# zailaiyiwan123/NOVA_pointcloud

Measured on AMD Instinct MI355X. Metric: generated points/sec/node, NOVA-d48w1024 @2048 pts, 64-step sample, higher is better.
Workload: dtype bf16; 1 GPU; d48w1024_2048pts_b32; ar_steps=64, diffusion_steps=25, batch_per_gpu=32, global_batch=32, guidance=cfg 2-pass, process_group=none

## Files before the change

include/nova_hip.h:

```cpp
#ifndef NOVA_HIP_H_
#define NOVA_HIP_H_

#ifdef __cplusplus
extern "C" {
#endif

#define NOVA_HIP_VERSION 405

typedef enum { NOVA_F32 = 0, NOVA_BF16 = 1, NOVA_F16 = 2 } nova_dtype;
typedef enum { NOVA_ACT_NONE = 0, NOVA_ACT_GELU_ERF = 1, NOVA_ACT_SILU = 2 } nova_act;
typedef enum {
  NOVA_OK = 0,
  NOVA_ERR_ARG = -1,
  NOVA_ERR_SHAPE = -2,
  NOVA_ERR_LAUNCH = -3,
  NOVA_ERR_DEVICE = -4
} nova_status;

int nova_version(void);
const char* nova_last_error(void);
int nova_check_device(void);

#define NOVA_PROF_SLOTS 10
int nova_prof_enable(int on);
int nova_prof_collect(double* ms, double* work, long long* launches, int slots);

int nova_debug_force_gemm_tile(int tile);

int nova_debug_set_attn_variant(int variant);

int nova_debug_set_graphs(int on);
int nova_debug_graph_stats(long* captures, long* replays);
int nova_debug_drop_graphs(void);

int nova_gemm_bias_act(const void* A, const void* W, const float* bias, void* out, int M, int N, int K, int act,
                       int dtype, void* stream);

int nova_quantize_rows_fp8(const void* x_bf16, void* out_fp8, float* scale, long long rows, int D, void* stream);
int nova_gemm_fp8_bias_act(const void* A8, const float* a_scale, const void* W8, const float* w_scale, const float* bias,
                           void* out_bf16, int M, int N, int K, int act, void* stream);

int nova_qkv_rope(const void* x, const void* Wqkv, const float* bias, const float* rope, void* qkv, int S, int L, int D,
                  int heads, int rope_batch, int dtype, void* stream);

int nova_qkv_rope_cols(const void* x, const void* W, const float* bias, const float* rope, void* out, int M, int N, int K,
                       int L, int rope_batch, int head_dim, int rope_cols, int dtype, void* stream);

int nova_rope_table(const float* pos, const long long* ids, float* rope, int nb, int pad, int n_tok, int n_pos, int hd,
                    const float* inv_freq, void* stream);

int nova_attn_fwd(const void* q, const void* k, const void* v, void* o, int S, int heads, int Lq, int Lk, int head_dim,
                  long q_row_stride, long kv_row_stride, long o_row_stride, float scale, int dtype, void* stream);

int nova_attn_fwd_lse(const void* q_scaled, const void* k, const void* v, void* o, float* lse, int S, int heads, int L,
                      int head_dim, long qkv_row_stride, long o_row_stride, const int* key_limit, void* stream);
int nova_attn_bwd(const void* q_scaled, const void* k, const void* v, const void* o, const void* d_o, const float* lse,
                  float* delta_scratch, void* dq, void* dk, void* dv, int S, int heads, int L, int head_dim,
                  long qkv_row_stride, long o_row_stride, long do_row_stride, long dqkv_row_stride, float scale,
                  const int* key_limit, void* stream);

int nova_attn_cross_fwd_lse(const void* q_scaled, const void* k, const void* v, void* o, float* lse, int S, int heads, int Lq, int Lk,
                            int head_dim, long q_row_stride, long kv_row_stride, long o_row_stride, const int* key_limit,
                            void* stream);
int nova_attn_cross_bwd(const void* q_scaled, const void* k, const void* v, const void* o, const void* d_o, const float* lse,
                        float* delta_scratch, void* dq, void* dk, void* dv, int S, int heads, int Lq, int Lk, int head_dim,
                        long q_row_stride, long kv_row_stride, long o_row_stride, long do_row_stride, long dq_row_stride,
                        long dkv_row_stride, float scale, const int* key_limit, void* stream);

int nova_act_fwd(const void* x, void* y, long long n, int kind, int dtype, void* stream);
int nova_act_bwd(const void* x, const void* dy, void* dx, long long n, int kind, int dtype, void* stream);

int nova_row_norm_bwd(const void* x, const void* dy, const float* gamma, const float* beta, const void* mod, long mod_ld,
                      int scale_off, int shift_off, int gate_off, void* dx, void* dmod, float* dgamma_part, float* dbeta_part,
                      int parts, long rows, int D, float eps, int dtype, void* stream);

int nova_row_norm(const void* in, void* out, const float* gamma, const float* beta, const void* mod, long mod_ld,
                  int scale_off, int shift_off, int gate_off, const void* res, const int* gather, long rows, int D,
                  float eps, int dtype, void* stream);

int nova_row_norm_chain(const void* g, const void* x, const float* gamma, const float* beta, const void* mod, long mod_ld,
// ... 227 lines not shown
```

nova_pointcloud_amd/csrc/capi.hip:

```cpp
#include <cstdarg>
#include <cstdio>
#include <cstring>
#include <atomic>
#include <cmath>
#include <mutex>
#include <utility>
#include <vector>
#include "common.h"
#include "nova_internal.h"

namespace nova {

static thread_local char g_err[512] = "";

int set_error(int code, const char* fmt, ...) {
  va_list ap;
  va_start(ap, fmt);
  vsnprintf(g_err, sizeof(g_err), fmt, ap);
  va_end(ap);
  return code;
}

int check_launch(const char* what) {
  const hipError_t e = hipGetLastError();
  if (e == hipSuccess) return 0;
  return set_error(NOVA_ERR_LAUNCH, "%s: %s", what, hipGetErrorString(e));
}

struct ProfRec { hipEvent_t a, b; int slot; double work; };
static std::atomic<bool> g_prof_on{false};
static std::mutex g_prof_mu;
static std::vector<ProfRec> g_prof;
static std::vector<std::pair<hipEvent_t, hipEvent_t>> g_prof_pool;

bool prof_enabled() { return g_prof_on.load(std::memory_order_relaxed); }

ProfScope::ProfScope(int slot, double work, hipStream_t s) : idx(-1), st(s) {
  if (!prof_enabled()) return;
  std::lock_guard<std::mutex> lk(g_prof_mu);
  ProfRec r;
  if (!g_prof_pool.empty()) {
    r.a = g_prof_pool.back().first;
    r.b = g_prof_pool.back().second;
    g_prof_pool.pop_back();
  } else if (hipEventCreate(&r.a) != hipSuccess || hipEventCreate(&r.b) != hipSuccess) {
    return;
  }
  r.slot = slot;
  r.work = work;
  (void)hipEventRecord(r.a, st);
  g_prof.push_back(r);
  idx = (int)g_prof.size() - 1;
}
ProfScope::~ProfScope() {
  if (idx < 0) return;
  std::lock_guard<std::mutex> lk(g_prof_mu);
  if (idx < (int)g_prof.size()) (void)hipEventRecord(g_prof[idx].b, st);
}

static thread_local bool g_walk_rev = false;
void walk_reverse(bool on) { g_walk_rev = on; }
bool walk_is_reverse() { return g_walk_rev; }
#ifdef NOVA_EXPERIMENTS
static int g_walk_alternate = 1;
void walk_set_alternate(int on) { g_walk_alternate = on; }
#else
constexpr int g_walk_alternate = 1;
#endif
struct Walk {
  int k = 0;
  void next() { walk_reverse(g_walk_alternate && (k++ & 1)); }
  ~Walk() { walk_reverse(false); }
};
}

using namespace nova;

extern "C" {

int nova_version(void) { return NOVA_HIP_VERSION; }
const char* nova_last_error(void) { return g_err; }

int nova_check_device(void) {
  int dev = -1;
  if (hipGetDevice(&dev) != hipSuccess) return set_error(NOVA_ERR_DEVICE, "no HIP device");
  hipDeviceProp_t prop;
  if (hipGetDeviceProperties(&prop, dev) != hipSuccess) return set_error(NOVA_ERR_DEVICE, "hipGetDeviceProperties failed");
  if (strncmp(prop.gcnArchName, "gfx950", 6) != 0)
    return set_error(NOVA_ERR_DEVICE, "device %d is %s; libnova_hip is built for gfx950 only", dev, prop.gcnArchName);
  return 0;
}

int nova_debug_force_gemm_tile(int tile) {
  NOVA_REQUIRE(gemm_force_tile(tile) == 0, NOVA_ERR_ARG,
               "force_gemm_tile: this build knows 0 (auto), 16 (small-M kernel; 161 / 162 / 164 with 16 / 32 / 64 rows per workgroup), 64 / 128 (the small-M tile kernels), 256 (persistent), 257 (one tile per workgroup) and 258 (persistent, prologue form); experiment codes need the NOVA_EXPERIMENTS build");
  return 0;
}

int nova_prof_enable(int on) {
  g_prof_on.store(on != 0);
  return 0;
}

int nova_prof_collect(double* ms, double* work, long long* launches, int slots) {
  NOVA_REQUIRE(ms && work && launches && slots >= PROF_SLOTS, NOVA_ERR_ARG, "prof_collect: need %d slots", PROF_SLOTS);
  for (int i = 0; i < slots; ++i) { ms[i] = 0; work[i] = 0; launches[i] = 0; }
  std::lock_guard<std::mutex> lk(g_prof_mu);
  for (auto& r : g_prof) {
    float t = 0.f;
    if (hipEventSynchronize(r.b) == hipSuccess && hipEventElapsedTime(&t, r.a, r.b) == hipSuccess) {
      ms[r.slot] += t;
      work[r.slot] += r.work;
      launches[r.slot] += 1;
    }
    g_prof_pool.emplace_back(r.a, r.b);
  }
  g_prof.clear();
  return 0;
}

int nova_gemm_bias_act(const void* A, const void* W, const float* bias, void* out, int M, int N, int K, int act,
                       int dtype, void* stream) {
  NOVA_REQUIRE(!bad_dtype(dtype), NOVA_ERR_ARG, "gemm: bad dtype %d", dtype);
  NOVA_REQUIRE(M == 0 || (A && W && out), NOVA_ERR_ARG, "gemm: null pointer");
  return gemm_bias_act(A, W, bias, out, M, N, K, act, dtype, (hipStream_t)stream);
}

int nova_quantize_rows_fp8(const void* x, void* out, float* scale, long long rows, int D, void* stream) {
  NOVA_REQUIRE(rows <= 0 || (x && out && scale), NOVA_ERR_ARG, "quantize_rows_fp8: null pointer");
  return quantize_rows_fp8(x, out, scale, (long)rows, D, (hipStream_t)stream);
}

int nova_gemm_fp8_bias_act(const void* A8, const float* a_scale, const void* W8, const float* w_scale, const float* bias,
                           void* out, int M, int N, int K, int act, void* stream) {
  NOVA_REQUIRE(M <= 0 || (A8 && a_scale && W8 && w_scale && out), NOVA_ERR_ARG, "gemm_fp8: null pointer");
  NOVA_REQUIRE(act >= NOVA_ACT_NONE && act <= NOVA_ACT_SILU, NOVA_ERR_ARG, "gemm_fp8: bad activation %d", act);
  return gemm256_fp8_launch({.A8 = A8, .sa = a_scale, .W8 = W8, .sw = w_scale, .C = out, .M = M, .N = N, .K = K, .epi = act, .e = epi_bias(bias)},
                            (hipStream_t)stream);
}

int nova_qkv_rope(const void* x, const void* Wqkv, const float* bias, const float* rope, void* qkv, int S, int L, int D,
                  int heads, int rope_batch, int dtype, void* stream) {
  NOVA_REQUIRE(!bad_dtype(dtype), NOVA_ERR_ARG, "qkv_rope: bad dtype %d", dtype);
  NOVA_REQUIRE(S * L == 0 || (x && Wqkv && qkv), NOVA_ERR_ARG, "qkv_rope: null pointer");
  return gemm_qkv_rope(x, Wqkv, bias, rope, qkv, S, L, D, heads, rope_batch, dtype, (hipStream_t)stream);
}

int nova_qkv_rope_cols(const void* x, const void* W, const float* bias, const float* rope, void* out, int M, int N, int K,
// ... 295 lines not shown
```

nova_pointcloud_amd/csrc/denoise.hip:

```cpp
#include <atomic>
#include <cstdlib>
#include <string>
#include <unordered_map>
#include <utility>
#include "nova_internal.h"

namespace nova {

enum class Echo { none, energy, rows };

struct DenoiseCall {
  const nova_decoder* dec;
  const void *zc, *temb;
  float* x;
  const nova_sampler_step* sched;
  const float *noise, *echo_noise;
  float renorm;
  Echo echo;
  float *echo_energy, *echo_rows;
  int Ne, steps, S, B, n, P, D;
  void *ws_a, *ws_u, *ws_h, *ws_f, *ws_g, *ws_mod;
  float* ws_v;
  int mod_steps, dtype;
  hipStream_t st;
// ... 103 lines not shown
      epoch = now;
    }
    auto it = execs.find(key);
    if (it == execs.end()) {
      if (execs.size() >= 2048) clear();
      hipGraphExec_t exec = nullptr;
      hipError_t e = hipStreamBeginCapture(st, hipStreamCaptureModeThreadLocal);
      if (e == hipSuccess) {
        const int rc = launches();
        hipGraph_t graph = nullptr;
        e = hipStreamEndCapture(st, &graph);
        if (e == hipSuccess && graph && rc == 0) e = hipGraphInstantiate(&exec, graph, nullptr, nullptr, 0);
        if (graph) (void)hipGraphDestroy(graph);
        if (rc != 0) return rc;
      }
      if (e != hipSuccess || !exec) {
        (void)hipGetLastError();
        return launches();
      }
      it = execs.emplace(std::move(key), exec).first;
      ++captures;
    } else {
      ++replays;
    }
    const hipError_t el = hipGraphLaunch(it->second, st);
    NOVA_REQUIRE(el == hipSuccess, NOVA_ERR_LAUNCH, "decoder_denoise: hipGraphLaunch failed: %s", hipGetErrorString(el));
    return 0;
  }
};
static thread_local DecoderGraphs g_dec_graphs;
static std::atomic<int> g_graphs_on{-1};

static bool graphs_enabled() {
  int v = g_graphs_on.load(std::memory_order_relaxed);
  if (v < 0) {
    const char* e = getenv("NOVA_GRAPHS");
    g_graphs_on.store(v = (e && e[0] == '0') ? 0 : 1);
  }
  return v != 0;
}

template <typename T> static void key_put(std::string& k, const T& v) { k.append(reinterpret_cast<const char*>(&v), sizeof(T)); }

static std::string graph_key(const DenoiseCall& c) {
  std::string key;
  key.reserve(512 + sizeof(nova_sampler_step) * c.steps + sizeof(nova_mlp_block) * c.dec->depth);
  key_put(key, c.dec->depth);
  const void* dec_ptrs[] = {c.dec->adaln_w, c.dec->adaln_b, c.dec->patch_w, c.dec->patch_b, c.dec->head_w, c.dec->head_b};
  key_put(key, dec_ptrs);
  for (int b = 0; b < c.dec->depth; ++b) key_put(key, c.dec->blocks[b]);
  for (int i = 0; i < c.steps; ++i) key_put(key, c.sched[i]);
  const void* ptrs[] = {c.zc, c.temb, c.x, c.ws_a, c.ws_u, c.ws_h, c.ws_f, c.ws_g, c.ws_mod, (const void*)c.st};
  key_put(key, ptrs);
  const int ints[] = {c.steps, c.S, c.B, c.n, c.P, c.D, c.mod_steps, c.dtype, walk_is_reverse() ? 1 : 0, gemm_forced_tile(), skinny_forced_row_blocks()};
  key_put(key, ints);
  return key;
}

static int denoise(const DenoiseCall& c) {
  if (c.n == 0 || c.B == 0) return 0;
  if (c.echo != Echo::none || !graphs_enabled() || prof_enabled() || c.noise != nullptr || c.steps < 2) return denoise_launches(c);
  return g_dec_graphs.run(graph_key(c), c.st, [&c] { return denoise_launches(c); });
}

}

using namespace nova;

extern "C" {

int nova_debug_set_graphs(int on) {
  g_graphs_on.store(on ? 1 : 0);
  if (!on) {
    g_graph_epoch.fetch_add(1);
    g_dec_graphs.clear();
  }
  return 0;
}

int nova_debug_drop_graphs(void) {
  g_dec_graphs.clear();
  return 0;
}

int nova_debug_graph_stats(long* captures, long* replays) {
  if (captures) *captures = g_dec_graphs.captures;
  if (replays) *replays = g_dec_graphs.replays;
  return 0;
}

int nova_decoder_denoise(const nova_decoder* dec, const void* zc, const void* temb, float* x, const nova_sampler_step* sched,
                         const float* noise, float renorm, float* echo_energy, int steps, int S, int B, int n, int P, int D,
                         void* ws_a, void* ws_u, void* ws_h, void* ws_f, void* ws_g, void* ws_mod, float* ws_v, int mod_steps,
                         int dtype, void* stream) {
  const DenoiseCall c{dec, zc, temb, x, sched, noise, nullptr, renorm, renorm < 1.0f ? Echo::energy : Echo::none, echo_energy, nullptr, 0,
                      steps, S, B, n, P, D, ws_a, ws_u, ws_h, ws_f, ws_g, ws_mod, ws_v, mod_steps, dtype, (hipStream_t)stream};
  NOVA_TRY(check_call("decoder_denoise", c));
  NOVA_REQUIRE(c.echo == Echo::none || (echo_energy && ws_v), NOVA_ERR_ARG, "decoder_denoise: renorm needs echo_energy and ws_v");
  return denoise(c);
}

int nova_decoder_denoise_echo(const nova_decoder* dec, const void* zc, const void* temb, float* x, const nova_sampler_step* sched,
                              const float* noise, float renorm, float* echo_rows, const float* echo_noise, int Ne, int steps, int S, int B,
                              int n, int P, int D, void* ws_a, void* ws_u, void* ws_h, void* ws_f, void* ws_g, void* ws_mod, float* ws_v,
                              int mod_steps, int dtype, void* stream) {
  const DenoiseCall c{dec, zc, temb, x, sched, noise, echo_noise, renorm, Echo::rows, nullptr, echo_rows, Ne,
                      steps, S, B, n, P, D, ws_a, ws_u, ws_h, ws_f, ws_g, ws_mod, ws_v, mod_steps, dtype, (hipStream_t)stream};
// ... 8 lines not shown
```

nova_pointcloud_amd/csrc/gemm.hip:

```cpp
#include <cstdlib>
#include "common.h"
#include "nova_internal.h"

namespace nova {

constexpr int ROWB = 128;

template <typename T> struct Frag;
template <> struct Frag<bf16_t> { u4v v; };
template <> struct Frag<f16_t> { u4v v; };
template <> struct Frag<float> { f4v v; };

__device__ __forceinline__ f4v mma(const Frag<bf16_t>& w, const Frag<bf16_t>& a, f4v c) { return Half16<bf16_t>::mfma16(w.v, a.v, c); }
__device__ __forceinline__ f4v mma(const Frag<f16_t>& w, const Frag<f16_t>& a, f4v c) { return Half16<f16_t>::mfma16(w.v, a.v, c); }
__device__ __forceinline__ f4v mma(const Frag<float>& w, const Frag<float>& a, f4v c) {
#pragma unroll
  for (int j = 0; j < 4; ++j) c = __builtin_amdgcn_mfma_f32_16x16x4f32(w.v[j], a.v[j], c, 0, 0, 0);
  return c;
}

template <typename T>
__device__ __forceinline__ Frag<T> lds_frag(const char* tile, int row, int chunk) {
  const int phys = chunk ^ ((row >> 1) & 7);
  Frag<T> f;
  f.v = *reinterpret_cast<const decltype(f.v)*>(tile + row * ROWB + phys * 16);
  return f;
}

#ifndef NOVA_GEMM64_STAGES
#define NOVA_GEMM64_STAGES 2
#endif
template <typename T, int EPI, int F = 4>
__global__ __launch_bounds__(256, 2) void gemm_kernel(const T* __restrict__ A, const T* __restrict__ W,
                                                       T* __restrict__ C, int M, int N, int K, int ntm,
                                                       int ntn, GemmEpi e) {
  constexpr int BM = 32 * F, BN = 32 * F, TILE_BYTES = BM * ROWB, WT = 16 * F;
  constexpr int NST = F == 2 ? NOVA_GEMM64_STAGES : 2;
  __shared__ __attribute__((aligned(16))) char smem[NST * 2 * TILE_BYTES];
  const int tid = threadIdx.x, lane = tid & 63, wid = tid >> 6;
  const int wm = wid >> 1, wn = wid & 1;

  int tm, tn;
  grouped_tile(xcd_remap(blockIdx.x, ntm * ntn), ntm, ntn, 8, tm, tn);
  const int m0 = tm * BM, n0 = tn * BN;

  const int rr = lane >> 3, cp = lane & 7;
  const char* a_src[4];
  const char* w_src[4];
  const size_t rowbytes = (size_t)K * sizeof(T);
#pragma unroll
  for (int i = 0; i < F; ++i) {
    const int row = (wid * F + i) * 8 + rr;
    const int c = cp ^ ((row >> 1) & 7);
    const int am = min(m0 + row, M - 1);
    a_src[i] = reinterpret_cast<const char*>(A) + (size_t)am * rowbytes + c * 16;
// ... 102 lines not shown
int gemm256_cu_count();

static thread_local int g_force_tile = 0;
#ifdef NOVA_EXPERIMENTS
void gemm256_set_variant(int v);
void gemm256_set_gm(int g);
void gemm256_set_stagger(int cycles);
void gemm256_set_grid(int n);
void walk_set_alternate(int on);
#endif
int gemm_forced_tile() { return g_force_tile; }
int gemm_force_tile(int tile) {
#ifdef NOVA_EXPERIMENTS
  if (tile == 50000 || tile == 50001) {
    walk_set_alternate(tile - 50000);
    return 0;
  }
  if (tile >= 40000 && tile <= 40512) {
    gemm256_set_grid(tile - 40000);
    return 0;
  }
  if (tile >= 30000 && tile < 31000) {
    gemm256_set_stagger((tile - 30000) * 256);
    return 0;
  }
  if (tile >= 7001 && tile <= 7064) {
    gemm256_set_gm(tile - 7000);
    return 0;
  }
  if (tile >= 2560 && tile <= 2580) {
    gemm256_set_variant(tile - 2560);
    tile = 256;
  }
#endif
  if (tile == 161 || tile == 162 || tile == 164) {
    skinny_force_row_blocks(tile - 160);
    tile = 16;
  } else {
    skinny_force_row_blocks(0);
  }
  if (tile != 0 && tile != 16 && tile != 64 && tile != 128 && tile != 256 && tile != 257 && tile != 258) return -1;
  g_force_tile = tile;
  return 0;
}

static long min_tiles256() {
  static const long v = [] {
    const char* e = getenv("NOVA_GEMM_MIN_TILES");
    return e && *e ? atol(e) : (long)gemm256_cu_count() / 2;
  }();
  return v;
}

template <typename T>
static int launch_gemm(const void* A, const void* W, void* C, int M, int N, int K, int epi, const GemmEpi& e,
                       hipStream_t st) {
  const int kelems = ROWB / (int)sizeof(T);
  if (M <= 0) return 0;
  if (N % 128 != 0 || K % kelems != 0 || K <= 0)
    return set_error(NOVA_ERR_SHAPE, "gemm: need N %% 128 == 0 and K %% %d == 0 (got M=%d N=%d K=%d)", kelems, M, N, K);
  const bool can256 = N % 256 == 0 && (epi != EPI_ROPE || (e.rope_cols % 256 == 0 && e.q_cols % 256 == 0));
  if (g_force_tile >= 256 && !can256) return set_error(NOVA_ERR_SHAPE, "gemm: 256-tile kernel needs N %% 256 == 0");
  const long tiles256 = (long)((M + 255) / 256) * (N / 256);
  if (can256 && (g_force_tile >= 256 || (g_force_tile == 0 && M >= 4096 && tiles256 >= min_tiles256())))
    return gemm256_launch(A, W, C, M, N, K, epi, e, dtype_of<T>(), st, g_force_tile == 257 ? 1 : g_force_tile == 258 ? 2 : 0);
  constexpr int BM = 128, BN = 128;
  int ntm = (M + BM - 1) / BM, ntn = N / BN;
  ProfScope prof(PROF_GEMM_SMALL, 2.0 * M * N * K, st);
  const T* a = static_cast<const T*>(A);
  const T* w = static_cast<const T*>(W);
  T* c = static_cast<T*>(C);
  static const bool tile64_ok = [] { const char* v = getenv("NOVA_GEMM_TILE64"); return !(v && v[0] == '0'); }();
  if (g_force_tile == 64 || (tile64_ok && g_force_tile == 0 && epi != EPI_ROPE && (long)ntm * ntn * 4 <= (long)gemm256_cu_count() * 3)) {
    if (epi == EPI_ROPE) return set_error(NOVA_ERR_SHAPE, "gemm: the 64 tile has no RoPE epilogue");
    ntm = (M + 63) / 64;
    ntn = N / 64;
    dim3 grid64(ntm * ntn), block(256);
    if (int rc = dispatch_epi(epi, [&](auto tag) {
          constexpr int EPI = decltype(tag)::value;
          if constexpr (EPI != EPI_ROPE) hipLaunchKernelGGL((gemm_kernel<T, EPI, 2>), grid64, block, 0, st, a, w, c, M, N, K, ntm, ntn, e);
        }))
      return rc;
    return check_launch("gemm (64 tile)");
  }
  dim3 grid(ntm * ntn), block(256);
  if (int rc = dispatch_epi(epi, [&](auto tag) {
        hipLaunchKernelGGL((gemm_kernel<T, decltype(tag)::value>), grid, block, 0, st, a, w, c, M, N, K, ntm, ntn, e);
      }))
    return rc;
  return check_launch("gemm");
}

int gemm_bias_act(const void* A, const void* W, const float* bias, void* out, int M, int N, int K, int act,
                  int dtype, hipStream_t st) {
  const GemmEpi e = epi_bias(bias);
  if (act < 0 || act > 2) return set_error(NOVA_ERR_ARG, "gemm: unknown activation %d", act);
  if (dtype_is16(dtype) && (g_force_tile == 16 || (g_force_tile == 0 && skinny_gemm_fits(M, N, K, false))))
    return skinny_gemm(A, W, bias, out, M, N, K, act, nullptr, dtype, st);
  return dispatch_dtype(dtype, [&](auto tag) { return launch_gemm<decltype(tag)>(A, W, out, M, N, K, act, e, st); });
}

bool gemm_modulate_fused(int M, int N, int K, int dtype) {
  return dtype_is16(dtype) && (g_force_tile == 16 || (g_force_tile == 0 && skinny_gemm_fits(M, N, K, true)));
}

int gemm_modulate_act(const RowNormArgs& pro, const void* W, const float* bias, void* out, int M, int N, int K, int act,
                      int dtype, hipStream_t st) {
  if (gemm_modulate_fused(M, N, K, dtype)) return skinny_gemm(nullptr, W, bias, out, M, N, K, act, &pro, dtype, st);
  if (int rc = row_norm(pro, dtype, st)) return rc;
  return gemm_bias_act(pro.out, W, bias, out, M, N, K, act, dtype, st);
}

int gemm_qkv_rope(const void* x, const void* Wqkv, const float* bias, const float* rope, void* qkv, int S, int L,
                  int D, int heads, int rope_batch, int dtype, hipStream_t st, float q_scale) {
  const int hd = D / heads;
  if (heads <= 0 || D % heads != 0 || hd % 4 != 0) return set_error(NOVA_ERR_SHAPE, "qkv_rope: bad heads/D");
  const int epi = (rope || q_scale != 1.0f) ? EPI_ROPE : EPI_NONE;
  if (rope && rope_batch <= 0) return set_error(NOVA_ERR_ARG, "qkv_rope: rope_batch must be > 0");
  const GemmEpi e = epi_qkv(bias, rope, L, rope_batch, hd, D, q_scale);
  return dispatch_dtype(dtype, [&](auto tag) { return launch_gemm<decltype(tag)>(x, Wqkv, qkv, S * L, 3 * D, D, epi, e, st); });
}

int gemm_rope_cols(const void* x, const void* W, const float* bias, const float* rope, void* out, int M, int N, int K,
                   int L, int rope_batch, int hd, int rope_cols, int dtype, hipStream_t st) {
  if (rope && rope_batch <= 0) return set_error(NOVA_ERR_ARG, "rope_cols: rope_batch must be > 0");
  GemmEpi e{bias, rope, L, rope ? rope_batch : 1, hd, rope_cols, 1.0f, 0};
  const int epi = rope ? EPI_ROPE : EPI_NONE;
  return dispatch_dtype(dtype, [&](auto tag) { return launch_gemm<decltype(tag)>(x, W, out, M, N, K, epi, e, st); });
}

}
```

nova_pointcloud_amd/csrc/nova_internal.h:

```cpp
#pragma once
#include <hip/hip_runtime.h>
#include <type_traits>
#include "../../include/nova_hip.h"

#include "common.h"

namespace nova {

template <typename T> constexpr int dtype_of() { return sizeof(T) == 4 ? NOVA_F32 : NOVA_BF16; }
template <> constexpr int dtype_of<f16_t>() { return NOVA_F16; }
inline bool dtype_is16(int dtype) { return dtype == NOVA_BF16 || dtype == NOVA_F16; }
template <typename F> inline auto dispatch_dtype(int dtype, F&& f) {
  return dtype == NOVA_BF16 ? f(bf16_t{}) : dtype == NOVA_F16 ? f(f16_t{}) : f(float{});
}
template <typename F> inline auto dispatch_half(int dtype, F&& f) { return dtype == NOVA_F16 ? f(f16_t{}) : f(bf16_t{}); }
inline bool bad_dtype(int dtype) { return dtype != NOVA_F32 && dtype != NOVA_BF16 && dtype != NOVA_F16; }
inline size_t esize(int dtype) { return dtype_is16(dtype) ? 2 : 4; }

int set_error(int code, const char* fmt, ...) __attribute__((format(printf, 2, 3)));
int check_launch(const char* what);
#define NOVA_REQUIRE(cond, code, ...) do { if (!(cond)) return set_error(code, __VA_ARGS__); } while (0)
#define NOVA_TRY(expr) do { const int rc_ = (expr); if (rc_ != 0) return rc_; } while (0)

enum { PROF_GEMM_NONE = 0, PROF_GEMM_GELU, PROF_GEMM_SILU, PROF_GEMM_ROPE, PROF_ATTN, PROF_ROWNORM, PROF_GEMM_SMALL, PROF_GEMM_WIDEK,
       PROF_TOKENS, PROF_DECODER, PROF_SLOTS };
inline int prof_gemm_slot(int epi, int N, int K) { return epi == 0 && K > N ? PROF_GEMM_WIDEK : PROF_GEMM_NONE + epi; }
struct ProfScope {
  ProfScope(int slot, double work, hipStream_t st);
  ~ProfScope();
  int idx;
  hipStream_t st;
};
bool prof_enabled();

struct GemmEpi {
  const float* bias;
  const float* rope;
  int L;
  int rope_batch;
  int hd;
  int rope_cols;
  float q_scale;
  int q_cols;
};
inline GemmEpi epi_bias(const float* bias) { return {bias, nullptr, 1, 1, 2, 0, 1.0f, 0}; }
inline GemmEpi epi_qkv(const float* bias, const float* rope, int L, int rope_batch, int hd, int D, float q_scale) {
  return {bias, rope, L, rope ? rope_batch : 1, hd, rope ? 2 * D : 0, q_scale, q_scale != 1.0f ? D : 0};
}
enum { EPI_NONE = 0, EPI_GELU = 1, EPI_SILU = 2, EPI_ROPE = 3, EPI_GELU_Q8 = 5 };
template <typename F> inline int dispatch_epi(int epi, F&& f) {
  switch (epi) {
    case EPI_NONE: f(std::integral_constant<int, EPI_NONE>{}); return 0;
    case EPI_GELU: f(std::integral_constant<int, EPI_GELU>{}); return 0;
    case EPI_SILU: f(std::integral_constant<int, EPI_SILU>{}); return 0;
    case EPI_ROPE: f(std::integral_constant<int, EPI_ROPE>{}); return 0;
    default: return set_error(NOVA_ERR_ARG, "gemm: unknown epilogue %d", epi);
  }
}
int gemm_bias_act(const void* A, const void* W, const float* bias, void* out, int M, int N, int K, int act,
                  int dtype, hipStream_t st);
int gemm_qkv_rope(const void* x, const void* Wqkv, const float* bias, const float* rope, void* qkv, int S, int L,
                  int D, int heads, int rope_batch, int dtype, hipStream_t st, float q_scale = 1.0f);

int gemm_rope_cols(const void* x, const void* W, const float* bias, const float* rope, void* out, int M, int N, int K,
                   int L, int rope_batch, int hd, int rope_cols, int dtype, hipStream_t st);
int gemm_force_tile(int tile);
int gemm_forced_tile();
void walk_reverse(bool on);
bool walk_is_reverse();

int attn_fwd(const void* q, const void* k, const void* v, void* o, int S, int heads, int Lq, int Lk, int hd,
             long q_row_stride, long kv_row_stride, long o_row_stride, float scale, int dtype, hipStream_t st,
             bool q_prescaled = false, long kv_seq_stride = 0, float* lse = nullptr, const int* klim = nullptr);
struct AttnFwdArgs {
  const void *q, *k, *v;
  void* o;
  int S, heads, Lq, Lk, hd;
  long q_rs, kv_rs, o_rs;
  float cl;
  int dtype;
  hipStream_t st;
  long kv_ss;
  float* lse;
  const int* klim;
};
template <typename E, typename K, typename... X> inline void attn_launch(K kernel, int rows_per_wg, const AttnFwdArgs& a, X... extra) {
  const int nq = (a.Lq + rows_per_wg - 1) / rows_per_wg;
  hipLaunchKernelGGL(kernel, dim3((unsigned)((long)nq * a.heads * a.S)), dim3(256), 0, a.st, (const E*)a.q, (const E*)a.k, (const E*)a.v, (E*)a.o,
                     a.Lq, a.Lk, a.q_rs, a.kv_rs, a.o_rs, a.cl, a.heads, nq, walk_is_reverse() ? 1 : 0, a.kv_ss, a.lse, extra...);
}
struct AttnForm {
  int mfma, nqb;
  bool summ, pipelined;
};
constexpr AttnForm ATTN_FORMS[6] = {{32, 2, false, false}, {16, 2, false, false}, {16, 4, false, false},
                                    {16, 2, true, false},  {16, 4, true, false},  {16, 4, true, true}};
constexpr int NOVA_ATTN_DEFAULT_VARIANT = 3;
int attn_fwd_m16(const AttnFwdArgs& a, AttnForm f);
int attn_set_variant(int v);
int attn_variant();
int attn_bwd(const void* q, const void* k, const void* v, const void* o, const void* d_o, const float* lse, float* delta, void* dq,
             void* dk, void* dv, int S, int heads, int Lq, int Lk, int hd, long q_rs, long kv_rs, long o_rs, long do_rs, long dq_rs,
             long dkv_rs, float scale, hipStream_t st,
             const int* klim = nullptr);

struct RowNormArgs {
  const void* in;
  void* out;
  const float* gamma;
  const float* beta;
  const void* mod;
  long mod_ld;
  int scale_off, shift_off, gate_off;
  const void* res;
  const int* gather;
  long rows;
  int D;
  float eps;
  int rev = 0;
  void* out8 = nullptr;
// ... 55 lines not shown
```

nova_pointcloud_amd/hip.py:

```python

import ctypes
import os
import threading

import torch

F32, BF16, F16 = 0, 1, 2
ACT_NONE, ACT_GELU_ERF, ACT_SILU = 0, 1, 2

_LIB_PATH = os.path.join(os.path.dirname(os.path.abspath(__file__)), "libnova_hip.so")
_lock = threading.Lock()
_lib = None
_device_ok = False

c_void_p, c_int, c_long, c_float = ctypes.c_void_p, ctypes.c_int, ctypes.c_long, ctypes.c_float


class NovaHipError(RuntimeError):
    """Raised when libnova_hip.so is missing, mis-built, or a call into it fails."""


class VitBlock(ctypes.Structure):

    _fields_ = [(k, c_void_p) for k in (
# ... 57 lines not shown
    "nova_pointset_pairwise_dist": [c_void_p] * 3 + [c_int] * 3 + [c_float, c_float, c_void_p],
    "nova_pointset_nearest_match": [c_void_p] * 4 + [c_int] * 3 + [c_float, c_float, c_int, c_void_p],
    "nova_pointset_nearest_match_bwd": [c_void_p] * 6 + [c_int] * 3 + [c_float, c_float, c_int, c_void_p],
    "nova_pointset_matched_dist": [c_void_p] * 4 + [c_int] * 2 + [c_float] * 3 + [c_void_p],
    "nova_pointset_matched_dist_bwd": [c_void_p] * 7 + [c_int] * 2 + [c_float] * 3 + [c_void_p],
    "nova_pointset_chamfer_matrix": [c_void_p] * 3 + [c_int] * 6 + [c_void_p],
    "nova_pointset_emd_matrix": [c_void_p] * 3 + [c_int] * 4 + [c_void_p],
    "nova_pointset_occupancy_grid": [c_void_p] * 5 + [c_int] * 5 + [c_void_p],
    "nova_pointset_farthest_point_sample": [c_void_p] * 4 + [c_int] * 3 + [c_void_p],
    "nova_pointset_knn": [c_void_p] * 4 + [c_int] * 5 + [c_void_p],
    "nova_pointset_neighbor_aggregate": [c_void_p] * 4 + [c_int] * 5 + [c_void_p],
    "nova_pointset_neighbor_inverse": [c_void_p] * 3 + [c_int] * 4 + [c_void_p],
    "nova_pointset_neighbor_aggregate_bwd": [c_void_p] * 8 + [c_int] * 5 + [c_void_p],
    "nova_pointset_kernel_interpolate": [c_void_p] * 4 + [c_int] * 4 + [c_float, c_void_p],
    "nova_pointset_kernel_interpolate_stats": [c_void_p] * 6 + [c_int] * 4 + [c_float, c_void_p],
    "nova_pointset_kernel_interpolate_bwd": [c_void_p] * 10 + [c_int] * 4 + [c_float, c_void_p],
    "nova_pointset_soft_cluster": [c_void_p] * 5 + [c_int] * 4 + [c_float, c_void_p],
    "nova_pointset_soft_cluster_bwd": [c_void_p] * 9 + [c_int] * 4 + [c_float, c_void_p],
    "nova_pointset_soft_cluster_sum_clouds": [c_void_p] * 2 + [c_int] * 2 + [c_void_p],
    "nova_pointset_posenc": [c_void_p] * 5 + [c_int] * 3 + [c_void_p],
    "nova_pointset_posenc_bwd": [c_void_p] * 7 + [c_int] * 3 + [c_void_p],
    "nova_pointset_embed": [c_void_p] * 7 + [c_int] * 4 + [c_void_p],
    "nova_pointset_embed_bwd": [c_void_p] * 7 + [c_int] * 4 + [c_void_p],
    "nova_pointset_embed_sum_clouds": [c_void_p] * 2 + [c_int] * 2 + [c_void_p],
    "nova_pointset_embed_pos_bwd": [c_void_p] * 2 + [c_int] * 4 + [c_void_p],
    "nova_pointset_head": [c_void_p, c_int] + [c_void_p] * 3 + [c_int] * 4 + [c_void_p],
    "nova_pointset_head_bwd": [c_void_p, c_int, c_void_p, c_void_p, c_float] + [c_void_p] * 4 + [c_int] * 4 + [c_void_p],
    "nova_bias_dropout_add": [c_void_p, c_int, c_void_p, c_void_p, c_void_p, ctypes.c_longlong, c_int, ctypes.c_longlong, ctypes.c_ulonglong, c_float,
                              ctypes.c_ulonglong, ctypes.c_ulonglong, c_int, c_void_p],
    "nova_bias_dropout_add_bwd": [c_void_p, c_void_p, c_int, c_void_p, c_void_p, ctypes.c_longlong, c_int, ctypes.c_longlong, ctypes.c_ulonglong, c_float,
                                  ctypes.c_ulonglong, ctypes.c_ulonglong, c_int, c_void_p],
    "nova_adamw_sumsq": [ctypes.POINTER(AdamWTensor), c_int, c_void_p, ctypes.c_longlong, c_void_p, c_void_p, c_void_p],
    "nova_adamw_step": [ctypes.POINTER(AdamWTensor), c_int, c_void_p, c_float, c_void_p],
    "nova_pointset_assignment": [c_void_p] * 5 + [c_int, c_int, c_float, c_float] + [c_int] * 3 + [c_void_p, c_void_p],
    "nova_pointset_assignment_rounds": [c_void_p, c_void_p, c_int, c_int, c_void_p],
    "nova_modulate_rows": [c_void_p] * 3 + [c_long, c_int, c_int, c_void_p],
    "nova_attn_fwd_lse": [c_void_p] * 5 + [c_int, c_int, c_int, c_int, c_long, c_long, c_void_p, c_void_p],
    "nova_attn_bwd": [c_void_p] * 10 + [c_int, c_int, c_int, c_int, c_long, c_long, c_long, c_long, c_float, c_void_p, c_void_p],
    "nova_attn_cross_fwd_lse": [c_void_p] * 5 + [c_int] * 5 + [c_long] * 3 + [c_void_p, c_void_p],
    "nova_attn_cross_bwd": [c_void_p] * 10 + [c_int] * 5 + [c_long] * 6 + [c_float, c_void_p, c_void_p],
    "nova_row_norm_bwd": [c_void_p] * 5 + [c_long, c_int, c_int, c_int] + [c_void_p] * 4 + [c_int, c_long, c_int, c_float, c_int, c_void_p],
    "nova_act_fwd": [c_void_p, c_void_p, ctypes.c_longlong, c_int, c_int, c_void_p],
    "nova_act_bwd": [c_void_p, c_void_p, c_void_p, ctypes.c_longlong, c_int, c_int, c_void_p],
    "nova_row_norm_chain": [c_void_p] * 5 + [c_long, c_int, c_int, c_int, c_float, c_float, c_void_p, c_void_p, c_long, c_int, c_int, c_void_p],
    "nova_adaln_fc1": [c_void_p, c_void_p, c_long, c_int, c_int, c_float, c_void_p, c_void_p, c_void_p, c_void_p, c_long]
    + [c_int] * 4 + [c_void_p],
    "nova_decoder_denoise": [ctypes.POINTER(Decoder), c_void_p, c_void_p, c_void_p, c_void_p, c_void_p, c_float, c_void_p]
    + [c_int] * 6 + [c_void_p] * 7 + [c_int, c_int, c_void_p],
    "nova_decoder_denoise_echo": [ctypes.POINTER(Decoder), c_void_p, c_void_p, c_void_p, c_void_p, c_void_p, c_float, c_void_p, c_void_p]
    + [c_int] * 7 + [c_void_p] * 7 + [c_int, c_int, c_void_p],
}
SIGNATURES["nova_prof_enable"] = [c_int]
SIGNATURES["nova_debug_force_gemm_tile"] = [c_int]
SIGNATURES["nova_debug_set_graphs"] = [c_int]
SIGNATURES["nova_debug_set_attn_variant"] = [c_int]
SIGNATURES["nova_debug_drop_graphs"] = []
SIGNATURES["nova_debug_graph_stats"] = [ctypes.POINTER(c_long), ctypes.POINTER(c_long)]
SIGNATURES["nova_prof_collect"] = [ctypes.POINTER(ctypes.c_double), ctypes.POINTER(ctypes.c_double),
                                   ctypes.POINTER(ctypes.c_longlong), c_int]
PROF_SLOTS = ["gemm_bias", "gemm_bias_gelu", "gemm_bias_silu", "qkv_gemm_rope", "attention", "row_norm", "gemm_small_tile", "gemm_bias_wide_k",
              "token_plumbing", "decoder_glue"]
PLAIN = {"nova_pointset_assignment_state_bytes": (ctypes.c_longlong, [c_int]), "nova_version": (c_int, []), "nova_last_error": (ctypes.c_char_p, []), "nova_check_device": (c_int, [])}


def lib_path() -> str:
    return _LIB_PATH


ABI_VERSION = 405


def load(check_device=True):
    global _lib, _device_ok
    with _lock:
        if _lib is None:
            if not os.path.exists(_LIB_PATH):
                raise NovaHipError(
                    f"{_LIB_PATH} not found: the HIP extension is not built. Run "
                    "`python -c 'import __graft_entry__ as g; g.build()'` (or `make -C nova_pointcloud_amd/csrc`). "
                    "There is no CPU fallback for the generation path."
                )
            try:
                lib = ctypes.CDLL(_LIB_PATH)
            except OSError as e:
                raise NovaHipError(f"cannot load {_LIB_PATH}: {e}") from e
            lib.nova_version.restype = c_int
            if lib.nova_version() != ABI_VERSION:
                raise NovaHipError(f"{_LIB_PATH} is C ABI version {lib.nova_version()}, this package binds version {ABI_VERSION} "
                                   "(include/nova_hip.h NOVA_HIP_VERSION): rebuild it with `make -C nova_pointcloud_amd/csrc`")
            try:
                for name, argtypes in SIGNATURES.items():
                    fn = getattr(lib, name)
                    fn.argtypes, fn.restype = argtypes, c_int
                for name, (res, argtypes) in PLAIN.items():
                    fn = getattr(lib, name)
                    fn.argtypes, fn.restype = argtypes, res
            except AttributeError as e:
                raise NovaHipError(f"{_LIB_PATH} lacks an entry point this package binds ({e}): rebuild it with "
                                   "`make -C nova_pointcloud_amd/csrc`") from e
            _lib = lib
        if check_device and not _device_ok:
            if not torch.cuda.is_available():
                raise NovaHipError("no GPU visible: libnova_hip needs an MI355X (gfx950) device")
            rc = _lib.nova_check_device()
            if rc != 0:
                raise NovaHipError(_lib.nova_last_error().decode())
# ... 108 lines not shown
    call("nova_qkv_rope_cols", ptr(x), ptr(w), ptr(bias, torch.float32), ptr(rope, torch.float32), ptr(out), M, N, K, L,
         rope.shape[0] if rope is not None else 1, hd, rope_cols, dtype_code(x.dtype), stream_ptr())
    return out


def modulate_rows(x, mod, out=None):
    rows, D = x.shape
    assert mod.shape == (rows, 2 * D) and mod.dtype == x.dtype
    out = torch.empty_like(x) if out is None else out
    call("nova_modulate_rows", ptr(x), ptr(mod), ptr(out), rows, D, dtype_code(x.dtype), stream_ptr())
    return out


def vit_blocks_forward_kv(blocks, x, S, L, heads, hidden, rope, cache, cache_cap, cache_len, ws_qkv, ws_a, ws_b, ws_h):
    D = x.shape[-1]
    call("nova_vit_blocks_forward_kv", blocks, len(blocks), ptr(x), S, L, D, heads, hidden, ptr(rope, torch.float32),
         rope.shape[0] if rope is not None else 1, ptr(cache), cache_cap, cache_len, ptr(ws_qkv), ptr(ws_a), ptr(ws_b),
         ptr(ws_h), dtype_code(x.dtype), stream_ptr())
    return x


def row_norm(x, out=None, gamma=None, beta=None, mod=None, scale_off=-1, shift_off=-1, gate_off=-1, res=None,
             gather=None, eps=1e-5, rows=None):
    D = x.shape[-1]
    rows = (gather.numel() if gather is not None else x.numel() // D) if rows is None else rows
    out = x.new_empty(rows, D) if out is None else out
    mod_ld = mod.shape[-1] if mod is not None else 0
    call("nova_row_norm", ptr(x), ptr(out), ptr(gamma, torch.float32), ptr(beta, torch.float32), ptr(mod), mod_ld,
         scale_off, shift_off, gate_off, ptr(res), ptr(gather, torch.int32), rows, D, float(eps),
         dtype_code(x.dtype), stream_ptr())
    return out


def adaln_fc1(x, mod, scale_off, shift_off, w, bias=None, act=ACT_SILU, eps=1e-6, out=None):
    rows, D = x.shape
    N = w.shape[0]
    out = x.new_empty(rows, N) if out is None else out
    h = x.new_empty(rows, D)
    call("nova_adaln_fc1", ptr(x), ptr(mod), mod.shape[-1], scale_off, shift_off, float(eps), ptr(w), ptr(bias, torch.float32),
         ptr(h), ptr(out), rows, N, D, act, dtype_code(x.dtype), stream_ptr())
    return out


def set_graphs(on=True):
    call("nova_debug_set_graphs", 1 if on else 0)


def graph_stats():
    c, r = c_long(0), c_long(0)
    call("nova_debug_graph_stats", ctypes.byref(c), ctypes.byref(r))
    return c.value, r.value


def prof_enable(on=True):
    call("nova_prof_enable", 1 if on else 0)


def prof_collect():
    n = len(PROF_SLOTS)
    ms, work, cnt = (ctypes.c_double * n)(), (ctypes.c_double * n)(), (ctypes.c_longlong * n)()
    call("nova_prof_collect", ms, work, cnt, n)
    return {PROF_SLOTS[i]: (ms[i], work[i], cnt[i]) for i in range(n)}
```

Baseline: 8195 points/s.

## Split large GEMMs into 256-tile main panels plus small-tile tail via cost model

```diff
diff --git a/include/nova_hip.h b/include/nova_hip.h
--- a/include/nova_hip.h
+++ b/include/nova_hip.h
@@ -26,6 +26,9 @@
 int nova_prof_collect(double* ms, double* work, long long* launches, int slots);
 
 int nova_debug_force_gemm_tile(int tile);
+
+int nova_debug_gemm_split(int mode);
+int nova_debug_gemm_split_stats(long* launches256, long* splits);
 
 int nova_debug_set_attn_variant(int variant);
 
diff --git a/nova_pointcloud_amd/csrc/capi.hip b/nova_pointcloud_amd/csrc/capi.hip
--- a/nova_pointcloud_amd/csrc/capi.hip
+++ b/nova_pointcloud_amd/csrc/capi.hip
@@ -32,11 +32,14 @@
 static std::mutex g_prof_mu;
 static std::vector<ProfRec> g_prof;
 static std::vector<std::pair<hipEvent_t, hipEvent_t>> g_prof_pool;
+static thread_local int g_prof_mute = 0;
+ProfMute::ProfMute() { ++g_prof_mute; }
+ProfMute::~ProfMute() { --g_prof_mute; }
 
 bool prof_enabled() { return g_prof_on.load(std::memory_order_relaxed); }
 
 ProfScope::ProfScope(int slot, double work, hipStream_t s) : idx(-1), st(s) {
-  if (!prof_enabled()) return;
+  if (!prof_enabled() || g_prof_mute > 0) return;
   std::lock_guard<std::mutex> lk(g_prof_mu);
   ProfRec r;
   if (!g_prof_pool.empty()) {
@@ -94,6 +97,16 @@
 int nova_debug_force_gemm_tile(int tile) {
   NOVA_REQUIRE(gemm_force_tile(tile) == 0, NOVA_ERR_ARG,
                "force_gemm_tile: this build knows 0 (auto), 16 (small-M kernel; 161 / 162 / 164 with 16 / 32 / 64 rows per workgroup), 64 / 128 (the small-M tile kernels), 256 (persistent), 257 (one tile per workgroup) and 258 (persistent, prologue form); experiment codes need the NOVA_EXPERIMENTS build");
+  return 0;
+}
+
+int nova_debug_gemm_split(int mode) {
+  NOVA_REQUIRE(gemm_set_split(mode) == 0, NOVA_ERR_ARG, "gemm_split: -1 (cost model), 0 (never) or a row-panel count > 0, got %d", mode);
+  return 0;
+}
+
+int nova_debug_gemm_split_stats(long* launches256, long* splits) {
+  gemm_split_stats(launches256, splits);
   return 0;
 }
 
diff --git a/nova_pointcloud_amd/csrc/denoise.hip b/nova_pointcloud_amd/csrc/denoise.hip
--- a/nova_pointcloud_amd/csrc/denoise.hip
+++ b/nova_pointcloud_amd/csrc/denoise.hip
@@ -179,7 +179,7 @@
   for (int i = 0; i < c.steps; ++i) key_put(key, c.sched[i]);
   const void* ptrs[] = {c.zc, c.temb, c.x, c.ws_a, c.ws_u, c.ws_h, c.ws_f, c.ws_g, c.ws_mod, (const void*)c.st};
   key_put(key, ptrs);
-  const int ints[] = {c.steps, c.S, c.B, c.n, c.P, c.D, c.mod_steps, c.dtype, walk_is_reverse() ? 1 : 0, gemm_forced_tile(), skinny_forced_row_blocks()};
+  const int ints[] = {c.steps, c.S, c.B, c.n, c.P, c.D, c.mod_steps, c.dtype, walk_is_reverse() ? 1 : 0, gemm_forced_tile(), skinny_forced_row_blocks(), gemm_split_mode()};
   key_put(key, ints);
   return key;
 }
diff --git a/nova_pointcloud_amd/csrc/gemm.hip b/nova_pointcloud_amd/csrc/gemm.hip
--- a/nova_pointcloud_amd/csrc/gemm.hip
+++ b/nova_pointcloud_amd/csrc/gemm.hip
@@ -1,6 +1,7 @@
 #include <cstdlib>
 #include "common.h"
 #include "nova_internal.h"
+#include "gemm_split.h"
 
 namespace nova {
 
@@ -209,26 +210,34 @@
   return v;
 }
 
+static thread_local int g_split_mode = -1;
+static thread_local long g_launches256 = 0, g_splits = 0;
+int gemm_set_split(int mode) {
+  if (mode < -1) return -1;
+  g_split_mode = mode;
+  return 0;
+}
+int gemm_split_mode() { return g_split_mode; }
+void gemm_split_stats(long* launches256, long* splits) {
+  if (launches256) *launches256 = g_launches256;
+  if (splits) *splits = g_splits;
+}
 template <typename T>
-static int launch_gemm(const void* A, const void* W, void* C, int M, int N, int K, int epi, const GemmEpi& e,
-                       hipStream_t st) {
-  const int kelems = ROWB / (int)sizeof(T);
-  if (M <= 0) return 0;
-  if (N % 128 != 0 || K % kelems != 0 || K <= 0)
-    return set_error(NOVA_ERR_SHAPE, "gemm: need N %% 128 == 0 and K %% %d == 0 (got M=%d N=%d K=%d)", kelems, M, N, K);
-  const bool can256 = N % 256 == 0 && (epi != EPI_ROPE || (e.rope_cols % 256 == 0 && e.q_cols % 256 == 0));
-  if (g_force_tile >= 256 && !can256) return set_error(NOVA_ERR_SHAPE, "gemm: 256-tile kernel needs N %% 256 == 0");
-  const long tiles256 = (long)((M + 255) / 256) * (N / 256);
-  if (can256 && (g_force_tile >= 256 || (g_force_tile == 0 && M >= 4096 && tiles256 >= min_tiles256())))
-    return gemm256_launch(A, W, C, M, N, K, epi, e, dtype_of<T>(), st, g_force_tile == 257 ? 1 : g_force_tile == 258 ? 2 : 0);
+static int split_panels(int M, int N, int K, int epi) {
+  static const bool env_on = [] { const char* v = getenv("NOVA_GEMM_SPLIT"); return !(v && v[0] == '0'); }();
+  const int p_total = (M + 255) / 256;
+  if (g_split_mode > 0) return g_split_mode < p_total ? g_split_mode : p_total;
+  if (g_split_mode == 0 || !env_on || sizeof(T) != 2) return p_total;
+  return gemm_split_plan(M, N, K, epi, gemm256_cu_count());
+}
+
+template <typename T>
+static int launch_small(const T* a, const T* w, T* c, int M, int N, int K, int epi, const GemmEpi& e, hipStream_t st, bool pick64) {
   constexpr int BM = 128, BN = 128;
   int ntm = (M + BM - 1) / BM, ntn = N / BN;
   ProfScope prof(PROF_GEMM_SMALL, 2.0 * M * N * K, st);
-  const T* a = static_cast<const T*>(A);
-  const T* w = static_cast<const T*>(W);
-  T* c = static_cast<T*>(C);
   static const bool tile64_ok = [] { const char* v = getenv("NOVA_GEMM_TILE64"); return !(v && v[0] == '0'); }();
-  if (g_force_tile == 64 || (tile64_ok && g_force_tile == 0 && epi != EPI_ROPE && (long)ntm * ntn * 4 <= (long)gemm256_cu_count() * 3)) {
+  if (g_force_tile == 64 || (tile64_ok && pick64 && epi != EPI_ROPE && (long)ntm * ntn * 4 <= (long)gemm256_cu_count() * 3)) {
     if (epi == EPI_ROPE) return set_error(NOVA_ERR_SHAPE, "gemm: the 64 tile has no RoPE epilogue");
     ntm = (M + 63) / 64;
     ntn = N / 64;
@@ -248,6 +257,41 @@
   return check_launch("gemm");
 }
 
+template <typename T>
+static int launch_gemm(const void* A, const void* W, void* C, int M, int N, int K, int epi, const GemmEpi& e,
+                       hipStream_t st) {
+  const int kelems = ROWB / (int)sizeof(T);
+  if (M <= 0) return 0;
+  if (N % 128 != 0 || K % kelems != 0 || K <= 0)
+    return set_error(NOVA_ERR_SHAPE, "gemm: need N %% 128 == 0 and K %% %d == 0 (got M=%d N=%d K=%d)", kelems, M, N, K);
+  const bool can256 = N % 256 == 0 && (epi != EPI_ROPE || (e.rope_cols % 256 == 0 && e.q_cols % 256 == 0));
+  if (g_force_tile >= 256 && !can256) return set_error(NOVA_ERR_SHAPE, "gemm: 256-tile kernel needs N %% 256 == 0");
+  const T* a = static_cast<const T*>(A);
+  const T* w = static_cast<const T*>(W);
+  T* c = static_cast<T*>(C);
+  const long tiles256 = (long)((M + 255) / 256) * (N / 256);
+  if (can256 && (g_force_tile >= 256 || (g_force_tile == 0 && M >= 4096 && tiles256 >= min_tiles256()))) {
+    const int form = g_force_tile == 257 ? 1 : g_force_tile == 258 ? 2 : 0;
+    const int p_total = (M + 255) / 256;
+    const int p_main = (epi != EPI_ROPE && form == 0) ? split_panels<T>(M, N, K, epi) : p_total;
+    ++g_launches256;
+    if (p_main >= p_total) return gemm256_launch(A, W, C, M, N, K, epi, e, dtype_of<T>(), st, form);
+    ++g_splits;
+    const int m_main = 256 * p_main;
+    ProfScope prof(prof_gemm_slot(epi, N, K), 2.0 * M * N * K, st);
+    ProfMute mute;
+    auto main = [&] { return gemm256_launch(A, W, C, m_main, N, K, epi, e, dtype_of<T>(), st, form); };
+    auto tail = [&] { return launch_small<T>(a + (size_t)m_main * K, w, c + (size_t)m_main * N, M - m_main, N, K, epi, e, st, true); };
+    if (walk_is_reverse()) {
+      if (int rc = tail()) return rc;
+      return main();
+    }
+    if (int rc = main()) return rc;
+    return tail();
+  }
+  return launch_small<T>(a, w, c, M, N, K, epi, e, st, g_force_tile == 0);
+}
+
 int gemm_bias_act(const void* A, const void* W, const float* bias, void* out, int M, int N, int K, int act,
                   int dtype, hipStream_t st) {
   const GemmEpi e = epi_bias(bias);
diff --git a/nova_pointcloud_amd/csrc/gemm_split.h b/nova_pointcloud_amd/csrc/gemm_split.h
--- /dev/null
+++ b/nova_pointcloud_amd/csrc/gemm_split.h
@@ -0,0 +1,53 @@
+#pragma once
+
+namespace nova {
+
+inline int gemm_split_rounds256(long tiles, int cus) {
+  const long chunk = (tiles + 7) / 8, nslot = cus / 8;
+  return (int)((chunk + nslot - 1) / nslot);
+}
+
+inline int gemm_split_tail_rounds(long rows, int N, int cus) {
+  const long tiles = ((rows + 127) / 128) * (N / 128);
+  return (int)((tiles + cus - 1) / cus);
+}
+
+struct GemmSplitRatio {
+  int N, K, epi;
+  double ratio;
+};
+constexpr GemmSplitRatio GEMM_SPLIT_RATIOS[] = {
+    {1024, 1024, 0, 0.77},
+    {1024, 4096, 0, 0.78},
+};
+constexpr double GEMM_SPLIT_MIN_GAIN = 0.1;
+constexpr int GEMM_SPLIT_MAX_ROUNDS = 5;
+
+inline double gemm_split_ratio(int N, int K, int epi) {
+  for (const GemmSplitRatio& r : GEMM_SPLIT_RATIOS)
+    if (r.N == N && r.K == K && r.epi == epi) return r.ratio;
+  return -1.0;
+}
+
+inline int gemm_split_plan_at(int M, int N, int cus, double ratio) {
+  const int p_total = (M + 255) / 256, ntn = N / 256;
+  if (ratio < 0 || ntn <= 0 || cus < 8) return p_total;
+  if (((long)p_total * ntn) % cus == 0) return p_total;
+  const int r_total = gemm_split_rounds256((long)p_total * ntn, cus);
+  if (r_total > GEMM_SPLIT_MAX_ROUNDS) return p_total;
+  int best = p_total;
+  double best_cost = r_total - GEMM_SPLIT_MIN_GAIN;
+  for (int r = 1; r < r_total; ++r) {
+    const int p = (int)((long)cus * r / ntn);
+    if (p <= 0 || p >= p_total) continue;
+    const double cost = gemm_split_rounds256((long)p * ntn, cus) + ratio * gemm_split_tail_rounds(M - 256L * p, N, cus);
+    if (cost < best_cost) {
+      best_cost = cost;
+      best = p;
+    }
+  }
+  return best;
+}
+inline int gemm_split_plan(int M, int N, int K, int epi, int cus) { return gemm_split_plan_at(M, N, cus, gemm_split_ratio(N, K, epi)); }
+
+}
diff --git a/nova_pointcloud_amd/csrc/nova_internal.h b/nova_pointcloud_amd/csrc/nova_internal.h
--- a/nova_pointcloud_amd/csrc/nova_internal.h
+++ b/nova_pointcloud_amd/csrc/nova_internal.h
@@ -30,6 +30,10 @@
   ~ProfScope();
   int idx;
   hipStream_t st;
+};
+struct ProfMute {
+  ProfMute();
+  ~ProfMute();
 };
 bool prof_enabled();
 
@@ -66,6 +70,9 @@
                    int L, int rope_batch, int hd, int rope_cols, int dtype, hipStream_t st);
 int gemm_force_tile(int tile);
 int gemm_forced_tile();
+int gemm_set_split(int mode);
+int gemm_split_mode();
+void gemm_split_stats(long* launches256, long* splits);
 void walk_reverse(bool on);
 bool walk_is_reverse();
 
diff --git a/nova_pointcloud_amd/hip.py b/nova_pointcloud_amd/hip.py
--- a/nova_pointcloud_amd/hip.py
+++ b/nova_pointcloud_amd/hip.py
@@ -133,6 +133,8 @@
 }
 SIGNATURES["nova_prof_enable"] = [c_int]
 SIGNATURES["nova_debug_force_gemm_tile"] = [c_int]
+SIGNATURES["nova_debug_gemm_split"] = [c_int]
+SIGNATURES["nova_debug_gemm_split_stats"] = [ctypes.POINTER(c_long), ctypes.POINTER(c_long)]
 SIGNATURES["nova_debug_set_graphs"] = [c_int]
 SIGNATURES["nova_debug_set_attn_variant"] = [c_int]
 SIGNATURES["nova_debug_drop_graphs"] = []
@@ -347,6 +349,16 @@
     return c.value, r.value
 
 
+def gemm_split(mode=-1):
+    call("nova_debug_gemm_split", int(mode))
+
+
+def gemm_split_stats():
+    n, s = c_long(0), c_long(0)
+    call("nova_debug_gemm_split_stats", ctypes.byref(n), ctypes.byref(s))
+    return n.value, s.value
+
+
 def prof_enable(on=True):
     call("nova_prof_enable", 1 if on else 0)
 
```

Result: no change. 8247 points/s (median of 6 runs) (+0.6%).
